# MarwanNour/SEAL-FYP-Logistic-Regression

Measured on AMD Instinct MI355X. Metric: CKKS ciphertext rotate+plain-mult ops/sec at N=16384; HBM GB/s vs roofline, higher is better.
Workload: dtype u64; 1 GPU; C3: N=16384, coeff_modulus bits [60, 40, 40, 40, 40, 60], level L=5 (k=6); per step and per GPU 4608 independent rotate_vector(step=1, direct Galois key)+multiply_plain, uniform random residues drawn on the device, inputs resident in HBM; batch_per_gpu=4608, parallelism=1 x independent ciphertext batches (no data-path collective), algorithmic_bytes_per_op=11141120

## Files before the change

### seal_fyp_logistic_regression_amd/csrc/hefx_keyswitch.hip

```cpp
#include <cstdio>
#include <cstdlib>
#include "hefx_internal.h"
#include "hefx_ntt.cuh"
#include "hefx_ntt8.cuh"

template <int LOGN>
struct KsWaves {
    static constexpr int INV = LOGN <= 14 ? 2 : 4;
    static constexpr int FWD = LOGN <= 13 ? 2 : 4;
    static constexpr int NB_INV = (INV <= 2 && LOGN <= 13) ? 1 : 2, NB_FWD = (FWD <= 2 && LOGN < 13) ? 1 : 2;
};

namespace hefx {

typedef u64 u64x2_t __attribute__((ext_vector_type(2)));
__device__ __forceinline__ ulonglong2 nt_load16(const u64 *p)
{
    const u64x2_t v = __builtin_nontemporal_load(reinterpret_cast<const u64x2_t *>(p));
    return make_ulonglong2(v.x, v.y);
}
__device__ __forceinline__ void nt_store16(u64 *p, u64 a, u64 b)
{
    u64x2_t v;
    v.x = a, v.y = b;
    __builtin_nontemporal_store(v, reinterpret_cast<u64x2_t *>(p));
}

template <int LOGN>
struct SplitCfg {
    using C = NttCfg<LOGN - 1>;
    static constexpr int N = 1 << LOGN;
    static constexpr int H = N / 2;
    static constexpr int T = C::T;
    static constexpr size_t LDS_BYTES = sizeof(u64) * C::LDS_WORDS;
};

__host__ __device__ static inline int split_grid(int rows) { return ((rows + 7) / 8) * 16; }
__device__ static __forceinline__ void split_decode(int bid, int &p, int &h)
{
    h = (bid >> 3) & 1;
    p = ((bid >> 4) << 3) | (bid & 7);
}
__host__ __device__ static inline int group_grid(int groups, int fan) { return ((groups + 7) / 8) * 2 * fan * 8; }
// ... 83 lines not shown
    extern __shared__ __align__(16) u64 lds[];
    int p, h;
    split_decode(blockIdx.x, p, h);
    if (p >= rows || (!noperm && ks_gated_out(S))) return;
    intt_digits_body<LOGN>(T, items[p / L], L, relin, noperm, p / L, p % L, h, S, lds);
}

#ifndef HEFX_SMALL_MAX
#define HEFX_SMALL_MAX 32
#endif
constexpr int KS_SMALL_MAX = HEFX_SMALL_MAX;
struct KsSmallItems {
    KsItem it[KS_SMALL_MAX];
};
static_assert(sizeof(KsSmallItems) + sizeof(DevTables) + sizeof(KsScratch) + sizeof(void *) + 8 * sizeof(int) <= 4096,
              "small-batch descriptors no longer fit the 4 KiB kernel-argument segment: lower HEFX_SMALL_MAX");
template <int LOGN>
__global__ __launch_bounds__(SplitCfg<LOGN>::T, KsWaves<LOGN>::INV) void ks_intt_digits_small_kernel(DevTables T, KsSmallItems small,
                                                                                    KsItem *__restrict__ items_out, int n,
                                                                                    int L, int relin, int rows, KsScratch S)
{
    extern __shared__ __align__(16) u64 lds[];
    HEFX_STAMP_KERNEL(0);
    HEFX_STAMP_AT(0);
    if (blockIdx.x == 0 && (int)threadIdx.x < n) items_out[threadIdx.x] = small.it[threadIdx.x];
    int p, h;
    split_decode(blockIdx.x, p, h);
    if (p >= rows) return;
    intt_digits_body<LOGN>(T, small.it[p / L], L, relin, 0, p / L, p % L, h, S, lds);
    HEFX_STAMP_AT(15);
}

__device__ __forceinline__ bool slot_is_f64(const DevTables &T, int L, int jj);
template <int LOGN>
__device__ __forceinline__ void ntt_digit_row(const DevTables &T, int L, int rows, int stream_x, const KsScratch &S,
                                              u64 *lds)
{
    using SC = SplitCfg<LOGN>;
    using C = typename SC::C;
    int g, jj, h;
    if (stream_x & 2) {
        const int x = blockIdx.x & 7, rest = blockIdx.x >> 3;
        const int nsg = (rows + 7) >> 3;
        const int sg = rest % nsg, slot = rest / nsg;
        g = sg * 8 + x;
        h = slot & 1;
        const int rank = slot >> 1, di = g % L;
        int heavy = 0;
        for (int mm = 0; mm < L; ++mm) heavy += !slot_is_f64(T, L, mm >= di ? mm + 1 : mm);
        int want = rank < heavy ? rank : rank - heavy;
        jj = 0;
        for (int mm = 0; mm < L; ++mm) {
            const bool hv = !slot_is_f64(T, L, mm >= di ? mm + 1 : mm);
            if (hv == (rank < heavy)) {
                if (want == 0) {
                    jj = mm;
                    break;
                }
                --want;
            }
        }
    } else
        group_decode(blockIdx.x, L, g, jj, h);
    if (g >= rows || (S.gate_mode == 2 && ks_gated_out(S))) return;
    const int t = threadIdx.x;
    const int b = g / L, i = g % L;
    if (jj >= i) ++jj;
    const int m = jj < L ? jj : T.k - 1;
    const ModConst mc = T.mods[m];
    const u64 qi = T.mods[i].q;
    const u64 *__restrict__ dd = S.d + ((size_t)b * L + i) * SC::N;
    u64 v[16];
    const InMode mode = {qi > mc.q, T.modsf[i].q == 0.0, false, 0};
    const int tl = HEFX_EO_LANE(SC, t);
    auto ld = [&](int r, u64 &x, u64 &y) {
        const uint32_t e = eo_nat<SC>(tl, r);
        x = dd[e];
        y = dd[e + SC::H / 2];
    };
    const ModConstF mf = T.modsf[m];
    split_fwd<LOGN, KsWaves<LOGN>::NB_FWD, true>(v, ld, mode, lds, ntt_tables(T, m), mc, mf, t, h, tl,
                                                 mac_x_slack(mc, mf, L));
    u64 *__restrict__ xd = S.x + (((size_t)b * L + i) * (L + 1) + jj) * SC::N + (size_t)h * SC::H;
    if (stream_x & 1) {
#pragma unroll
        for (int r = 0; r < 16; r += 2) nt_store16(xd + C::idx_io(t, r), v[r], v[r + 1]);
    } else {
#pragma unroll
        for (int r = 0; r < 16; r += 2)
            *reinterpret_cast<ulonglong2 *>(xd + C::idx_io(t, r)) = make_ulonglong2(v[r], v[r + 1]);
    }
}

struct MacW {
    struct Ctx {
        ModConst mc;
    };
    __device__ static __forceinline__ Ctx make(const ModConst &mc, const ModConstF &) { return Ctx{mc}; }
    typedef ulonglong2 X;
    struct K {
        ulonglong2 k0, k1;
    };
    __device__ static __forceinline__ X xin(const ulonglong2 &bits, bool, const Ctx &) { return bits; }
    __device__ static __forceinline__ K kin(const ulonglong2 &k0, const ulonglong2 &k1, const Ctx &) { return K{k0, k1}; }
    u64 a0xl = 0, a0xh = 0, a0yl = 0, a0yh = 0, a1xl = 0, a1xh = 0, a1yl = 0, a1yh = 0;
    __device__ __forceinline__ void mac(const X &x, const K &k, const Ctx &)
    {
        mac128(a0xl, a0xh, x.x, k.k0.x);
        mac128(a0yl, a0yh, x.y, k.k0.y);
        mac128(a1xl, a1xh, x.x, k.k1.x);
        mac128(a1yl, a1yh, x.y, k.k1.y);
    }
    __device__ __forceinline__ void mac_diag(const MacW &in, const ulonglong2 &dg, const Ctx &c)
    {
        ulonglong2 r0, r1;
        in.result(r0, r1, c);
        mac128(a0xl, a0xh, r0.x, dg.x);
        mac128(a0yl, a0yh, r0.y, dg.y);
        mac128(a1xl, a1xh, r1.x, dg.x);
        mac128(a1yl, a1yh, r1.y, dg.y);
    }
    template <bool LT2Q = false>
    __device__ __forceinline__ void result_data(ulonglong2 &r0, ulonglong2 &r1, const Ctx &c) const { result<LT2Q>(r0, r1, c); }
    template <bool LT2Q = false>
    __device__ __forceinline__ void result(ulonglong2 &r0, ulonglong2 &r1, const Ctx &c) const
    {
        r0.x = LT2Q ? barrett128_lt2q(a0xl, a0xh, c.mc) : barrett128(a0xl, a0xh, c.mc);
        r0.y = LT2Q ? barrett128_lt2q(a0yl, a0yh, c.mc) : barrett128(a0yl, a0yh, c.mc);
        r1.x = LT2Q ? barrett128_lt2q(a1xl, a1xh, c.mc) : barrett128(a1xl, a1xh, c.mc);
        r1.y = LT2Q ? barrett128_lt2q(a1yl, a1yh, c.mc) : barrett128(a1yl, a1yh, c.mc);
    }
};

struct MacL {
    typedef MacW::Ctx Ctx;
    __device__ static __forceinline__ Ctx make(const ModConst &mc, const ModConstF &) { return Ctx{mc}; }
    struct X {
        uint32_t xl, xh, yl, yh;
    };
    struct K {
        uint32_t k0xl, k0xh, k0yl, k0yh, k1xl, k1xh, k1yl, k1yh;
    };
    __device__ static __forceinline__ uint32_t lo30(u64 v) { return (uint32_t)v & 0x3FFFFFFFu; }
    __device__ static __forceinline__ uint32_t hi30(u64 v) { return (uint32_t)(v >> 30); }
    __device__ static __forceinline__ X xin(const ulonglong2 &b, bool, const Ctx &)
    {
        return X{lo30(b.x), hi30(b.x), lo30(b.y), hi30(b.y)};
    }
    __device__ static __forceinline__ K kin(const ulonglong2 &k0, const ulonglong2 &k1, const Ctx &)
    {
        return K{lo30(k0.x), hi30(k0.x), lo30(k0.y), hi30(k0.y), lo30(k1.x), hi30(k1.x), lo30(k1.y), hi30(k1.y)};
    }
    u64 c[4][3] = {};
    __device__ static __forceinline__ void mad(u64 (&col)[3], uint32_t xl, uint32_t xh, uint32_t kl, uint32_t kh)
    {
        col[0] += (u64)xl * kl;
        col[1] += (u64)xl * kh;
        col[1] += (u64)xh * kl;
        col[2] += (u64)xh * kh;
    }
    __device__ __forceinline__ void mac(const X &x, const K &k, const Ctx &)
    {
        mad(c[0], x.xl, x.xh, k.k0xl, k.k0xh);
        mad(c[1], x.yl, x.yh, k.k0yl, k.k0yh);
        mad(c[2], x.xl, x.xh, k.k1xl, k.k1xh);
        mad(c[3], x.yl, x.yh, k.k1yl, k.k1yh);
    }
    __device__ __forceinline__ void mac_diag(const MacL &in, const ulonglong2 &dg, const Ctx &cx)
    {
        ulonglong2 r0, r1;
        in.result(r0, r1, cx);
        const uint32_t dxl = lo30(dg.x), dxh = hi30(dg.x), dyl = lo30(dg.y), dyh = hi30(dg.y);
        mad(c[0], lo30(r0.x), hi30(r0.x), dxl, dxh);
        mad(c[1], lo30(r0.y), hi30(r0.y), dyl, dyh);
        mad(c[2], lo30(r1.x), hi30(r1.x), dxl, dxh);
        mad(c[3], lo30(r1.y), hi30(r1.y), dyl, dyh);
    }
    template <bool LT2Q>
    __device__ static __forceinline__ u64 fold(const u64 (&col)[3], const ModConst &mc)
    {
        u64 lo = col[0], hi = 0, t = col[1] << 30;
        lo += t;
        hi += (col[1] >> 34) + (lo < t);
        t = col[2] << 60;
        lo += t;
        hi += (col[2] >> 4) + (lo < t);
        return LT2Q ? barrett128_lt2q(lo, hi, mc) : barrett128(lo, hi, mc);
    }
    template <bool LT2Q = false>
    __device__ __forceinline__ void result_data(ulonglong2 &r0, ulonglong2 &r1, const Ctx &cx) const { result<LT2Q>(r0, r1, cx); }
    template <bool LT2Q = false>
    __device__ __forceinline__ void result(ulonglong2 &r0, ulonglong2 &r1, const Ctx &cx) const
    {
        r0.x = fold<LT2Q>(c[0], cx.mc);
        r0.y = fold<LT2Q>(c[1], cx.mc);
        r1.x = fold<LT2Q>(c[2], cx.mc);
        r1.y = fold<LT2Q>(c[3], cx.mc);
    }
};

struct MacF {
    typedef ArithF64::Ctx Ctx;
    __device__ static __forceinline__ Ctx make(const ModConst &, const ModConstF &mf) { return ArithF64::make(mf); }
    typedef double2 X;
    struct K {
        double k0x, k0y, k1x, k1y;
    };
    __device__ static __forceinline__ X xin(const ulonglong2 &b, bool own, const Ctx &)
    {
        return own ? make_double2(ArithF64::from_u64(b.x), ArithF64::from_u64(b.y))
                   : make_double2(__longlong_as_double((long long)b.x), __longlong_as_double((long long)b.y));
    }
    __device__ static __forceinline__ K kin(const ulonglong2 &k0, const ulonglong2 &k1, const Ctx &)
    {
        return K{ArithF64::from_u64(k0.x), ArithF64::from_u64(k0.y), ArithF64::from_u64(k1.x), ArithF64::from_u64(k1.y)};
    }
    double a0x = 0.0, a0y = 0.0, a1x = 0.0, a1y = 0.0;
    __device__ __forceinline__ void mac(const X &x, const K &k, const Ctx &c)
    {
        a0x += ArithF64::mm(x.x, k.k0x, c);
        a0y += ArithF64::mm(x.y, k.k0y, c);
        a1x += ArithF64::mm(x.x, k.k1x, c);
        a1y += ArithF64::mm(x.y, k.k1y, c);
    }
    __device__ __forceinline__ void mac_diag(const MacF &in, const ulonglong2 &dg, const Ctx &c)
    {
        const double dx = ArithF64::from_u64(dg.x), dy = ArithF64::from_u64(dg.y);
        a0x += ArithF64::mm(in.a0x, dx, c);
        a0y += ArithF64::mm(in.a0y, dy, c);
        a1x += ArithF64::mm(in.a1x, dx, c);
        a1y += ArithF64::mm(in.a1y, dy, c);
    }
    template <bool LT2Q = false>
    __device__ __forceinline__ void result_data(ulonglong2 &r0, ulonglong2 &r1, const Ctx &) const
    {
        r0.x = ArithF64::raw(a0x), r0.y = ArithF64::raw(a0y), r1.x = ArithF64::raw(a1x), r1.y = ArithF64::raw(a1y);
    }
    template <bool LT2Q = false>
    __device__ __forceinline__ void result(ulonglong2 &r0, ulonglong2 &r1, const Ctx &c) const
    {
        r0.x = ArithF64::canon(a0x, c);
        r0.y = ArithF64::canon(a0y, c);
        r1.x = ArithF64::canon(a1x, c);
        r1.y = ArithF64::canon(a1y, c);
    }
};

__device__ __forceinline__ bool slot_is_f64(const DevTables &T, int L, int jj)
{
    return T.modsf[jj < L ? jj : T.k - 1].q != 0.0;
}

template <class F>
__device__ __forceinline__ void mac_dispatch(const DevTables &T, int m, int L, const F &f)
{
    if (T.modsf[m].q != 0.0)
        f(MacF());
    else if (L <= 8 && (T.mods[m].q >> 60) == 0)
        f(MacL());
    else
        f(MacW());
}

template <bool STREAM>
__device__ __forceinline__ void mac_store(u64 *acc0, u64 *acc1, size_t w, const ulonglong2 &r0, const ulonglong2 &r1)
{
    if (STREAM) {
        nt_store16(acc0 + 2 * w, r0.x, r0.y);
        nt_store16(acc1 + 2 * w, r1.x, r1.y);
    } else {
        gst16(acc0 + 2 * w, r0);
        gst16(acc1 + 2 * w, r1);
    }
}

template <class P, int NI, bool STREAM, class XR>
__device__ __forceinline__ void mac_items(const DevTables &T, const u64 *key, int L, int jj, int m, size_t n, size_t w,
                                          const u64 *const (&own)[NI], const uint32_t (&own_elt)[NI], const XR &xrow,
                                          u64 *const (&acc0)[NI], u64 *const (&acc1)[NI])
{
    const typename P::Ctx cx = P::make(T.mods[m], T.modsf[m]);
    const int logn = T.logn;
    const size_t kpoly = (size_t)T.k * n;
    P A[NI];
    auto load_k = [&](int i, ulonglong2 &k0, ulonglong2 &k1) {
        const u64 *kb = key + ((size_t)i * 2 * T.k + m) * n;
        k0 = gld16(kb + 2 * w);
        k1 = gld16(kb + kpoly + 2 * w);
    };
    auto load_x = [&](int i, ulonglong2 (&xb)[NI]) {
#pragma unroll
        for (int e = 0; e < NI; ++e) {
            const u64 *xp = xrow(e, i) + 2 * w;
            xb[e] = STREAM ? nt_load16(xp) : gld16(xp);
        }
    };
    if (jj < L) {
        ulonglong2 xb[NI], k0, k1;
#pragma unroll
        for (int e = 0; e < NI; ++e) xb[e] = gather_pair(own[e], (uint32_t)w, own_elt[e], logn);
        load_k(jj, k0, k1);
        const typename P::K k = P::kin(k0, k1, cx);
#pragma unroll
        for (int e = 0; e < NI; ++e) A[e].mac(P::xin(xb[e], true, cx), k, cx);
    }
    constexpr int G = 1;
    auto digit_at = [&](int r) { return r < jj ? r : r + 1; };
    const int nd = jj < L ? L - 1 : L;
    int r0 = 0;
    for (; r0 + G <= nd; r0 += G) {
        ulonglong2 xb[G][NI], k0[G], k1[G];
#pragma unroll
        for (int g = 0; g < G; ++g) {
            load_x(digit_at(r0 + g), xb[g]);
            load_k(digit_at(r0 + g), k0[g], k1[g]);
        }
        HEFX_STAGE_FENCE();
#pragma unroll
        for (int g = 0; g < G; ++g) {
            const typename P::K k = P::kin(k0[g], k1[g], cx);
#pragma unroll
            for (int e = 0; e < NI; ++e) A[e].mac(P::xin(xb[g][e], false, cx), k, cx);
        }
    }
    for (; r0 < nd; ++r0) {
        ulonglong2 xb[NI], k0, k1;
        load_x(digit_at(r0), xb);
        load_k(digit_at(r0), k0, k1);
        const typename P::K k = P::kin(k0, k1, cx);
#pragma unroll
        for (int e = 0; e < NI; ++e) A[e].mac(P::xin(xb[e], false, cx), k, cx);
    }
#pragma unroll
    for (int e = 0; e < NI; ++e) {
        ulonglong2 r0, r1;
        if (jj < L)
            A[e].template result_data<true>(r0, r1, cx);
        else
            A[e].template result<true>(r0, r1, cx);
        mac_store<STREAM>(acc0[e], acc1[e], w, r0, r1);
    }
}

template <bool STREAM>
__device__ __forceinline__ void mac_unit(const DevTables &T, const KsItem *__restrict__ items, int L, int relin, int count,
                                         const KsScratch &S, int jj, int bl0, size_t w)
{
    const size_t n = (size_t)1 << T.logn;
    const int m = jj < L ? jj : T.k - 1;
    const bool two = bl0 + 1 < count;
    const KsItem it0 = items[bl0], it1 = items[bl0 + (two ? 1 : 0)];
    const int ownrow = jj < L ? jj : 0;
    const u64 *const own[2] = {it0.c_in + ((size_t)(relin ? 2 * L : L) + ownrow) * n,
                               it1.c_in + ((size_t)(relin ? 2 * L : L) + ownrow) * n};
    const uint32_t own_elt[2] = {relin ? 1u : item_elt(it0), relin ? 1u : item_elt(it1)};
    auto xrow2 = [&](int e, int i) { return S.x + (((size_t)(bl0 + e) * L + i) * (L + 1) + jj) * n; };
    auto accrow = [&](int bl, int c) { return S.acc + (((size_t)bl * 2 + c) * (L + 1) + jj) * n; };
    u64 *const acc0[2] = {accrow(bl0, 0), accrow(bl0 + 1, 0)}, *const acc1[2] = {accrow(bl0, 1), accrow(bl0 + 1, 1)};
    mac_dispatch(T, m, L, [&](auto pol) {
        using P = decltype(pol);
        if (two && it1.key == it0.key) {
            mac_items<P, 2, STREAM>(T, it0.key, L, jj, m, n, w, own, own_elt, xrow2, acc0, acc1);
        } else {
            const u64 *const o0[1] = {own[0]}, *const o1[1] = {own[1]};
            const uint32_t e0[1] = {own_elt[0]}, e1[1] = {own_elt[1]};
            u64 *const a00[1] = {acc0[0]}, *const a01[1] = {acc1[0]}, *const a10[1] = {acc0[1]}, *const a11[1] = {acc1[1]};
            mac_items<P, 1, STREAM>(T, it0.key, L, jj, m, n, w, o0, e0, [&](int, int i) { return xrow2(0, i); }, a00, a01);
            if (two)
                mac_items<P, 1, STREAM>(T, it1.key, L, jj, m, n, w, o1, e1, [&](int, int i) { return xrow2(1, i); }, a10, a11);
        }
    });
}

template <bool STREAM>
__global__ __launch_bounds__(256) void ks_mac_kernel(DevTables T, const KsItem *__restrict__ items, int L, int relin,
                                                     int count, KsScratch S)
{
    if (S.gate_mode == 2 && ks_gated_out(S)) return;
    const int jj = blockIdx.y;
#ifdef HEFX_STAMP
    const int wg = blockIdx.x + gridDim.x * (blockIdx.y + gridDim.y * blockIdx.z);
    if (threadIdx.x == 0 && wg < 1024) hefx_stamp_buf[((size_t)2 * 1024 + wg) * 16] = wall_clock64();
#endif
    mac_unit<STREAM>(T, items, L, relin, count, S, jj, 2 * blockIdx.z, (size_t)blockIdx.x * blockDim.x + threadIdx.x);
#ifdef HEFX_STAMP
    if (HEFX_STAMP > 1) asm volatile("s_waitcnt vmcnt(0) lgkmcnt(0)" ::: "memory");
    if (threadIdx.x == 0 && wg < 1024) hefx_stamp_buf[((size_t)2 * 1024 + wg) * 16 + 15] = wall_clock64();
#endif
}

template <int LOGN>
__global__ __launch_bounds__(SplitCfg<LOGN>::T, KsWaves<LOGN>::FWD) void ks_ntt_digits_kernel(DevTables T, int L, int rows,
                                                                             int stream_x, KsScratch S)
{
    extern __shared__ __align__(16) u64 lds[];
    HEFX_STAMP_KERNEL(1);
    HEFX_STAMP_AT(0);
    ntt_digit_row<LOGN>(T, L, rows, stream_x, S, lds);
    HEFX_STAMP_AT(15);
}

template <class P>
__device__ __forceinline__ void mac_gathered(P &A, const typename P::Ctx &cx, const DevTables &T, const KsItem &it,
                                             const u64 *__restrict__ c1, const KsScratch &S, int L, int jj, int m,
                                             size_t n, size_t w)
{
    const uint2 pi = gld_u32x2(it.perm + 2 * w);
    for (int i = 0; i < L; ++i) {
        const u64 *__restrict__ xrow = i == jj ? c1 + (size_t)i * n : S.x + ((size_t)i * (L + 1) + jj) * n;
        ulonglong2 xb;
        xb.x = gld8(xrow + pi.x);
        xb.y = gld8(xrow + pi.y);
        const u64 *kbase = it.key + ((size_t)i * 2 * T.k + m) * n;
        const ulonglong2 k0 = gld16(kbase + 2 * w);
        const ulonglong2 k1 = gld16(kbase + (size_t)T.k * n + 2 * w);
        A.mac(P::xin(xb, i == jj, cx), P::kin(k0, k1, cx), cx);
    }
}

__global__ __launch_bounds__(256) void ks_mac_exact_kernel(DevTables T, const KsItem *__restrict__ items, int L, KsScratch S)
{
    const size_t n = (size_t)1 << T.logn;
    const int jj = blockIdx.y, b = blockIdx.z;
    const int m = jj < L ? jj : T.k - 1;
    const size_t w = (size_t)blockIdx.x * blockDim.x + threadIdx.x;
    const KsItem it = items[b];
    if (w == 0 && jj == 0 && b == 0 && *S.gate == S.gate_tag) atomicAdd(S.gate_hits, 1u);
    const u64 *__restrict__ c1 = it.c_in + (size_t)L * n;
    const u64 *__restrict__ xs = S.x + (size_t)it.dsrc * L * (L + 1) * n;
    mac_dispatch(T, m, L, [&](auto pol) {
        using P = decltype(pol);
// ... 822 lines not shown
    }
}

template <int LOGN>
__global__ __launch_bounds__(256) void ks_pair_finish_kernel(DevTables T, const KsItem *__restrict__ items, int L, int relin,
                                                            KsScratch S)
{
    const int row = blockIdx.y, b = blockIdx.z;
    const int c = row / L, j = row % L;
    const uint32_t g = blockIdx.x * blockDim.x + threadIdx.x;
#ifdef HEFX_STAMP
    const int wg = blockIdx.x + gridDim.x * (blockIdx.y + gridDim.y * blockIdx.z);
    if (threadIdx.x == 0 && wg < 1024) hefx_stamp_buf[((size_t)5 * 1024 + wg) * 16] = wall_clock64();
#endif
    const KsItem it = items[b];
    const ModConst mc = T.mods[j];
    fwd_policy_dispatch(mc, T.modsf[j], [&](auto pol) {
        using A = decltype(pol);
        pair_finish_body<LOGN, A>(T, it, L, relin, b, c, j, g, S);
    });
#ifdef HEFX_STAMP
    if (HEFX_STAMP > 1) asm volatile("s_waitcnt vmcnt(0) lgkmcnt(0)" ::: "memory");
    if (threadIdx.x == 0 && wg < 1024) hefx_stamp_buf[((size_t)5 * 1024 + wg) * 16 + 15] = wall_clock64();
#endif
}

template <typename K>
static void set_lds(K kernel, size_t bytes)
{
    (void)hipFuncSetAttribute(reinterpret_cast<const void *>(kernel), hipFuncAttributeMaxDynamicSharedMemorySize,
                              (int)bytes);
}

template <int LOGN>
static hipError_t launch_keyswitch_chunk_t(const DevTables &T, int L, int n, const KsItem *batch, bool relin,
                                           const KsScratch &scr, bool alias, const KsSmallItems *small, int quarter,
                                           hipStream_t s, KsProf *prof, int nsrc)
{
    using SC = SplitCfg<LOGN>;
    const size_t lds = SC::LDS_BYTES;
    static PerDeviceOnce attr_once;
    if (attr_once.first()) {
        set_lds(ks_intt_digits_kernel<LOGN>, lds);
        set_lds(ks_intt_digits_small_kernel<LOGN>, lds);
        set_lds(ks_ntt_digits_kernel<LOGN>, lds);
        set_lds(ks_moddown_intt_kernel<LOGN>, lds);
        set_lds(ks_moddown_finish_kernel<LOGN>, lds);
        if (getenv("HEFX_DEBUG")) {
            int nb = -1;
            (void)hipOccupancyMaxActiveBlocksPerMultiprocessor(&nb, ks_ntt_digits_kernel<LOGN>, SC::T, lds);
            fprintf(stderr, "[hefx] ks_ntt_digits_kernel<%d>: %d threads, %zu B LDS -> %d workgroups/CU\n", LOGN, SC::T,
                    lds, nb);
        }
    }
    const int rl = relin ? 1 : 0;
    auto mark = [&](int stage) {
        if (prof && prof->used < prof->cap) {
            (void)hipEventRecord(prof->ev[prof->used], s);
            prof->stage[prof->used++] = stage;
        }
    };
    if (nsrc > 0) {
        KsScratch hs = scr, fb = scr;
        hs.gate_mode = 1;
        fb.gate_mode = 2;
        mark(1);
        hipLaunchKernelGGL((ks_intt_digits_kernel<LOGN>), dim3(split_grid(nsrc * L)), dim3(SC::T), lds, s, T, batch + n, L,
                           0, 1, nsrc * L, hs);
        mark(2);
        hipLaunchKernelGGL((ks_ntt_digits_kernel<LOGN>), dim3(group_grid(nsrc * L, L)), dim3(SC::T), lds, s, T, L, nsrc * L, 0,
                           hs);
        mark(3);
        hipLaunchKernelGGL(ks_mac_exact_kernel, dim3(SC::N / 2 / 256, L + 1, n), dim3(256), 0, s, T, batch, L, hs);
        mark(4);
        hipLaunchKernelGGL((ks_moddown_intt_kernel<LOGN>), dim3(split_grid(n * 2)), dim3(SC::T), lds, s, T, L, n * 2, hs);
        mark(5);
        hipLaunchKernelGGL((ks_moddown_finish_kernel<LOGN>), dim3(group_grid(n * 2, L)), dim3(SC::T), lds, s, T, batch, L,
                           0, n * 2, hs);
        mark(7);
        hipLaunchKernelGGL((ks_intt_digits_kernel<LOGN>), dim3(split_grid(n * L)), dim3(SC::T), lds, s, T, batch, L, 0, 0,
                           n * L, fb);
        hipLaunchKernelGGL((ks_ntt_digits_kernel<LOGN>), dim3(group_grid(n * L, L)), dim3(SC::T), lds, s, T, L, n * L, 0, fb);
        hipLaunchKernelGGL(ks_mac_kernel<false>, dim3(SC::N / 2 / 256, L + 1, (n + 1) / 2), dim3(256), 0, s, T, batch, L, 0, n,
                           fb);
        hipLaunchKernelGGL((ks_moddown_intt_kernel<LOGN>), dim3(split_grid(n * 2)), dim3(SC::T), lds, s, T, L, n * 2, fb);
// ... 13 lines not shown
        mark(1);
        hipLaunchKernelGGL((ks_pair_digits_kernel<LOGN>), fan_grid(n * L, 4 * L), dim3(TQ), ldsq, s, T, *small,
                           const_cast<KsItem *>(batch), n, L, rl, n * L, scr);
        mark(3);
        hipLaunchKernelGGL((ks_pair_mac_kernel<LOGN>), dim3(SC::N / 4 / 256, 2 * (L + 1), n), dim3(256), 0, s, T, batch, L, rl,
                           scr);
        mark(4);
        hipLaunchKernelGGL((ks_pair_moddown_kernel<LOGN>), fan_grid(n * 2, 4 * L), dim3(TQ), ldsq, s, T, L, n * 2,
                           scr);
        mark(5);
        hipLaunchKernelGGL((ks_pair_finish_kernel<LOGN>), dim3(SC::N / 4 / 256, 2 * L, n), dim3(256), 0, s, T, batch, L, rl,
                           scr);
        mark(-1);
        return hipGetLastError();
    }
    const int heavy_order = n * L * L * 2 <= 640 ? 2 : 0;
    if (small && (quarter & KS_Q_ALL)) {
        static PerDeviceOnce attrq;
        const size_t ldsq = QuarterCfg<LOGN>::LDS_BYTES;
        if (attrq.first()) {
            set_lds(ks_intt_digits_q_kernel<LOGN>, ldsq);
            set_lds(ks_ntt_digits_q_kernel<LOGN>, ldsq);
            set_lds(ks_moddown_intt_q_kernel<LOGN>, ldsq);
            set_lds(ks_moddown_finish_q_kernel<LOGN>, ldsq);
        }
        constexpr int TQ = QuarterCfg<LOGN>::T;
        mark(1);
        if (quarter & KS_Q_INTT)
            hipLaunchKernelGGL((ks_intt_digits_q_kernel<LOGN>), dim3(quarter_grid(n * L)), dim3(TQ), ldsq, s, T, *small,
                               const_cast<KsItem *>(batch), n, L, rl, n * L, scr);
        else
            hipLaunchKernelGGL((ks_intt_digits_small_kernel<LOGN>), dim3(split_grid(n * L)), dim3(SC::T), lds, s, T, *small,
                               const_cast<KsItem *>(batch), n, L, rl, n * L, scr);
        mark(2);
        if (quarter & KS_Q_NTT)
            hipLaunchKernelGGL((ks_ntt_digits_q_kernel<LOGN>), fan_grid(n * L, 4 * L), dim3(TQ), ldsq, s, T, L,
                               n * L, scr);
        else
            hipLaunchKernelGGL((ks_ntt_digits_kernel<LOGN>), dim3(group_grid(n * L, L)), dim3(SC::T), lds, s, T, L,
                               n * L, heavy_order, scr);
        mark(3);
        hipLaunchKernelGGL(ks_mac_kernel<false>, dim3(SC::N / 2 / 256, L + 1, (n + 1) / 2), dim3(256), 0, s, T, batch, L, rl, n,
                           scr);
        mark(4);
        if (quarter & KS_Q_MDI)
            hipLaunchKernelGGL((ks_moddown_intt_q_kernel<LOGN>), dim3(quarter_grid(n * 2)), dim3(TQ), ldsq, s, T, L, n * 2,
                               scr);
        else
            hipLaunchKernelGGL((ks_moddown_intt_kernel<LOGN>), dim3(split_grid(n * 2)), dim3(SC::T), lds, s, T, L, n * 2,
                               scr);
        mark(5);
        if (quarter & KS_Q_FIN)
            hipLaunchKernelGGL((ks_moddown_finish_q_kernel<LOGN>), fan_grid(n * 2, 4 * L), dim3(TQ), ldsq, s, T,
                               batch, L, rl, n * 2, scr);
        else
            hipLaunchKernelGGL((ks_moddown_finish_kernel<LOGN>), dim3(group_grid(n * 2, L)), dim3(SC::T), lds, s, T,
                               batch, L, rl, n * 2, scr);
        mark(-1);
        return hipGetLastError();
    }
    if (alias) {
        mark(0);
        hipLaunchKernelGGL(ks_alias_copy_kernel, dim3(SC::N / 2 / 256, 2 * L, n), dim3(256), 0, s, T, batch, L);
    }
    mark(1);
    if (small)
        hipLaunchKernelGGL((ks_intt_digits_small_kernel<LOGN>), dim3(split_grid(n * L)), dim3(SC::T), lds, s, T, *small,
                           const_cast<KsItem *>(batch), n, L, rl, n * L, scr);
    else
        hipLaunchKernelGGL((ks_intt_digits_kernel<LOGN>), dim3(split_grid(n * L)), dim3(SC::T), lds, s, T, batch, L, rl, 0,
                           n * L, scr);
    mark(2);
    const int stream_x = (size_t)n * L * (L + 1) * SC::N * 8 > ((size_t)256 << 20) ? 1 : 0;
    hipLaunchKernelGGL((ks_ntt_digits_kernel<LOGN>), dim3(group_grid(n * L, L)), dim3(SC::T), lds, s, T, L, n * L,
                       stream_x | heavy_order, scr);
    mark(3);
    if (stream_x)
        hipLaunchKernelGGL(ks_mac_kernel<true>, dim3(SC::N / 2 / 256, L + 1, (n + 1) / 2), dim3(256), 0, s, T, batch, L, rl, n,
                           scr);
    else
        hipLaunchKernelGGL(ks_mac_kernel<false>, dim3(SC::N / 2 / 256, L + 1, (n + 1) / 2), dim3(256), 0, s, T, batch, L, rl, n,
                           scr);
    mark(4);
    hipLaunchKernelGGL((ks_moddown_intt_kernel<LOGN>), dim3(split_grid(n * 2)), dim3(SC::T), lds, s, T, L, n * 2, scr);
    mark(5);
    hipLaunchKernelGGL((ks_moddown_finish_kernel<LOGN>), dim3(group_grid(n * 2, L)), dim3(SC::T), lds, s, T, batch, L,
                       rl, n * 2, scr);
    mark(-1);
    return hipGetLastError();
}

__global__ __launch_bounds__(256) void lt2_reduce_kernel(DevTables T, int L, int period, int rows, int chunks,
                                                         const u64 *__restrict__ partial, const u64 *addin, u64 *out)
{
    const size_t n = (size_t)1 << T.logn;
    const int r = blockIdx.y;
    const int jj = r % period;
    const u64 q = T.mods[jj < L ? jj : T.k - 1].q;
    const size_t w = (size_t)blockIdx.x * blockDim.x + threadIdx.x;
    ulonglong2 acc = addin ? reinterpret_cast<const ulonglong2 *>(addin + (size_t)r * n)[w] : make_ulonglong2(0, 0);
    for (int ch = 0; ch < chunks; ++ch) {
        const ulonglong2 v = reinterpret_cast<const ulonglong2 *>(partial + ((size_t)ch * rows + r) * n)[w];
        acc.x = addmod(acc.x, v.x, q);
        acc.y = addmod(acc.y, v.y, q);
    }
    if (period == L + 1 && jj < L && T.modsf[jj].q != 0.0)
        acc = make_ulonglong2(ArithF64::raw(ArithF64::from_u64(acc.x)), ArithF64::raw(ArithF64::from_u64(acc.y)));
    reinterpret_cast<ulonglong2 *>(out + (size_t)r * n)[w] = acc;
}

template <int LOGN>
static hipError_t launch_lt2_decompose_t(const DevTables &T, int L, const KsItem *src_item, const KsItem *rot_items,
                                         int nrot, const KsScratch &scr, const u64 *ct_new, u64 *partial_s,
                                         u64 *partial_c0, u64 *cbuf, hipStream_t s)
{
// ... 265 lines not shown
```

### seal_fyp_logistic_regression_amd/csrc/hefx_ntt.cuh

```cuda
#pragma once
#include <type_traits>

#include "hefx_modarith.cuh"

#ifdef HEFX_STAMP
namespace hefx {
static __device__ u64 hefx_stamp_buf[8 * 1024 * 16];
__device__ __forceinline__ int &hefx_stamp_kid()
{
    __shared__ int kid;
    return kid;
}
}
#define HEFX_STAMP_KERNEL(k) do { if (threadIdx.x == 0) hefx_stamp_kid() = (k); } while (0)
#define HEFX_STAMP_AT(id)                                                                                            \
    do {                                                                                                             \
        if (HEFX_STAMP > 1) asm volatile("s_waitcnt vmcnt(0) lgkmcnt(0)" ::: "memory");                              \
        const unsigned hefx_wg_ = blockIdx.x + gridDim.x * (blockIdx.y + gridDim.y * blockIdx.z);                   \
        if (threadIdx.x == 0 && hefx_wg_ < 1024)                                                                     \
            hefx_stamp_buf[((size_t)hefx_stamp_kid() * 1024 + hefx_wg_) * 16 + (id)] = wall_clock64();               \
    } while (0)
#else
#define HEFX_STAMP_KERNEL(k) do { } while (0)
#define HEFX_STAMP_AT(id) do { } while (0)
// ... 607 lines not shown
                                            u64 *lds, const typename A::TW *__restrict__ tw,
                                            const typename A::Ctx &cx, int t, int h, int t0 = -1, int mac_slack = 0)
{
    typename A::V f[16];
    split_fwd_raw<LOGN, A, LD, NB>(f, ld, mode, mc, lds, tw, cx, t, h, NoHook(), t0);
    if (MACOP && !A::IS_F64 && mac_slack == 1) {
#pragma unroll
        for (int r = 0; r < 16; ++r) v[r] = A::template mac_operand_lazy<1>(f[r], cx);
    } else if (MACOP && !A::IS_F64 && mac_slack >= 2) {
#pragma unroll
        for (int r = 0; r < 16; ++r) v[r] = A::template mac_operand_lazy<2>(f[r], cx);
    } else {
#pragma unroll
        for (int r = 0; r < 16; ++r) v[r] = MACOP ? A::mac_operand(f[r], cx) : A::fwd_finish(f[r], cx);
    }
}

template <int LOGN, int NB = 2, bool MACOP = false, class LD>
__device__ __forceinline__ void split_fwd(u64 (&v)[16], const LD &ld, const InMode &mode, u64 *lds,
                                          const NttTables &nt, const ModConst &mc, const ModConstF &mf, int t, int h,
                                          int t0 = -1, int mac_slack = 0)
{
    if (mf.q != 0.0)
        split_fwd_a<LOGN, ArithF64, LD, NB, MACOP>(v, ld, mode, mc, lds, nt.twf, ArithF64::make(mf), t, h, t0);
    else if constexpr (MACOP)
        fwd_int_dispatch(mc, [&](auto pol) {
            using A = decltype(pol);
            split_fwd_a<LOGN, A, LD, NB, MACOP>(v, ld, mode, mc, lds, nt.tw, A::make(mc), t, h, t0, mac_slack);
        });
    else
        split_fwd_a<LOGN, ArithU64, LD, NB, MACOP>(v, ld, mode, mc, lds, nt.tw, ArithU64::make(mc), t, h, t0);
}

template <int LOGN, class A, int NB = 2, class LDP>
__device__ __forceinline__ void split_inv_a(u64 (&v)[16], const LDP &ldp, u64 *lds,
                                            const typename A::TW *__restrict__ itw, const typename A::Ctx &cx, int t,
                                            int h)
{
    using C = NttCfg<LOGN - 1>;
    constexpr int BS = 16 / NB;
    typename A::V f[16];
    constexpr bool NATREC = C::R != 1;
    auto rec = [&](int r) { return NATREC ? C::idx_nat(t, r) : C::idx_out(t, r); };
#pragma unroll
    for (int g = 0; g < NB; ++g) {
        ulonglong2 pr[BS];
#pragma unroll
        for (int r = 0; r < BS; ++r) pr[r] = ldp(rec(BS * g + r));
        if (h == 0) {
#pragma unroll
            for (int r = 0; r < BS; ++r)
                f[BS * g + r] = A::gs_half_sum(A::from_u64(pr[r].x), A::from_u64(pr[r].y), cx);
        } else {
            typename A::TW w[BS];
#pragma unroll
            for (int r = 0; r < BS; ++r) w[r] = itw[C::N + rec(BS * g + r)];
#pragma unroll
            for (int r = 0; r < BS; ++r)
                f[BS * g + r] = A::gs_half_diff(A::from_u64(pr[r].x), A::from_u64(pr[r].y), w[r], cx);
        }
        HEFX_STAGE_FENCE();
    }
    if constexpr (C::R == 0) {
        typename A::V *lf = reinterpret_cast<typename A::V *>(lds);
        const int pw = t + (t >> 4), pr = 17 * t;
#pragma unroll
// ... 36 lines not shown
```

Measured before the change: 232,700 rotate+multiply_plain ops/s.

## Split digit forward NTT by parity and fuse last butterfly into MAC

The key-switch digit NTT now runs two independent half-size NTTs per digit, one per parity half (parity_fwd), with no cross-half exchange. The final radix-2 stage is deferred into the MAC kernel: each lane swaps its value with the neighbouring lane via DPP, then applies the last Cooley-Tukey butterfly with the matching twiddle before accumulating against the key. This removes the split-NTT cross-half exchange and its LDS traffic. In exchange the MAC kernel does extra butterfly arithmetic and lane shuffles for each digit element.

```diff
diff --git a/seal_fyp_logistic_regression_amd/csrc/hefx_keyswitch.hip b/seal_fyp_logistic_regression_amd/csrc/hefx_keyswitch.hip
--- a/seal_fyp_logistic_regression_amd/csrc/hefx_keyswitch.hip
+++ b/seal_fyp_logistic_regression_amd/csrc/hefx_keyswitch.hip
@@ -9,6 +9,7 @@
     static constexpr int INV = LOGN <= 14 ? 2 : 4;
     static constexpr int FWD = LOGN <= 13 ? 2 : 4;
     static constexpr int NB_INV = (INV <= 2 && LOGN <= 13) ? 1 : 2, NB_FWD = (FWD <= 2 && LOGN < 13) ? 1 : 2;
+    static constexpr bool PARITY_CUT = true;
 };
 
 namespace hefx {
@@ -158,7 +159,8 @@
 }
 
 __device__ __forceinline__ bool slot_is_f64(const DevTables &T, int L, int jj);
-template <int LOGN>
+__device__ __forceinline__ int mac_kind(const DevTables &T, int m, int L);
+template <int LOGN, bool CUT>
 __device__ __forceinline__ void ntt_digit_row(const DevTables &T, int L, int rows, int stream_x, const KsScratch &S,
                                               u64 *lds)
 {
@@ -198,15 +200,21 @@
     const u64 *__restrict__ dd = S.d + ((size_t)b * L + i) * SC::N;
     u64 v[16];
     const InMode mode = {qi > mc.q, T.modsf[i].q == 0.0, false, 0};
-    const int tl = HEFX_EO_LANE(SC, t);
-    auto ld = [&](int r, u64 &x, u64 &y) {
-        const uint32_t e = eo_nat<SC>(tl, r);
-        x = dd[e];
-        y = dd[e + SC::H / 2];
-    };
     const ModConstF mf = T.modsf[m];
-    split_fwd<LOGN, KsWaves<LOGN>::NB_FWD, true>(v, ld, mode, lds, ntt_tables(T, m), mc, mf, t, h, tl,
-                                                 mac_x_slack(mc, mf, L));
+    if constexpr (CUT) {
+        const u64 *__restrict__ dh = dd + (size_t)h * SC::H;
+        parity_fwd<LOGN>(v, [&](int r) { return dh[C::idx_nat(t, r)]; }, mode, lds, ntt_tables(T, m), mc, mf, t,
+                         mac_kind(T, m, L));
+    } else {
+        const int tl = HEFX_EO_LANE(SC, t);
+        auto ld = [&](int r, u64 &x, u64 &y) {
+            const uint32_t e = eo_nat<SC>(tl, r);
+            x = dd[e];
+            y = dd[e + SC::H / 2];
+        };
+        split_fwd<LOGN, KsWaves<LOGN>::NB_FWD, true>(v, ld, mode, lds, ntt_tables(T, m), mc, mf, t, h, tl,
+                                                     mac_x_slack(mc, mf, L));
+    }
     u64 *__restrict__ xd = S.x + (((size_t)b * L + i) * (L + 1) + jj) * SC::N + (size_t)h * SC::H;
     if (stream_x & 1) {
 #pragma unroll
@@ -229,6 +237,14 @@
     };
     __device__ static __forceinline__ X xin(const ulonglong2 &bits, bool, const Ctx &) { return bits; }
     __device__ static __forceinline__ K kin(const ulonglong2 &k0, const ulonglong2 &k1, const Ctx &) { return K{k0, k1}; }
+    typedef ulonglong2 LTW;
+    __device__ static __forceinline__ LTW ltw(const NttTables &nt, size_t i) { return gld16(nt.tw + i); }
+    __device__ static __forceinline__ X xin_cut(u64 e, u64 o, const LTW &w, const Ctx &c, int)
+    {
+        const ArithU64::Ctx ac = ArithU64::make(c.mc);
+        ArithU64::ct(e, o, w, ac, 0);
+        return make_ulonglong2(ArithU64::fwd_finish(e, ac), ArithU64::fwd_finish(o, ac));
+    }
     u64 a0xl = 0, a0xh = 0, a0yl = 0, a0yh = 0, a1xl = 0, a1xh = 0, a1yl = 0, a1yh = 0;
     __device__ __forceinline__ void mac(const X &x, const K &k, const Ctx &)
     {
@@ -277,6 +293,21 @@
     {
         return K{lo30(k0.x), hi30(k0.x), lo30(k0.y), hi30(k0.y), lo30(k1.x), hi30(k1.x), lo30(k1.y), hi30(k1.y)};
     }
+    typedef ulonglong2 LTW;
+    __device__ static __forceinline__ LTW ltw(const NttTables &nt, size_t i) { return gld16(nt.tw + i); }
+    __device__ static __forceinline__ u64 cut_reduce(u64 x, const ArithU64L::Ctx &ac, int slack)
+    {
+        x = csubn(csubn(x, ac.n8q), ac.n4q);
+        if (slack < 2) x = csubn(x, ac.n2q);
+        if (slack < 1) x = csubn(x, ac.nq);
+        return x;
+    }
+    __device__ static __forceinline__ X xin_cut(u64 e, u64 o, const LTW &w, const Ctx &c, int slack)
+    {
+        const ArithU64L::Ctx ac = ArithU64L::make(c.mc);
+        ArithU64L::ct(e, o, w, ac, 1);
+        return xin(make_ulonglong2(cut_reduce(e, ac, slack), cut_reduce(o, ac, slack)), false, c);
+    }
     u64 c[4][3] = {};
     __device__ static __forceinline__ void mad(u64 (&col)[3], uint32_t xl, uint32_t xh, uint32_t kl, uint32_t kh)
     {
@@ -341,6 +372,14 @@
     {
         return K{ArithF64::from_u64(k0.x), ArithF64::from_u64(k0.y), ArithF64::from_u64(k1.x), ArithF64::from_u64(k1.y)};
     }
+    typedef double LTW;
+    __device__ static __forceinline__ LTW ltw(const NttTables &nt, size_t i) { return nt.twf[i]; }
+    __device__ static __forceinline__ X xin_cut(u64 e, u64 o, const LTW &w, const Ctx &c, int)
+    {
+        double x = ArithF64::unraw(e), y = ArithF64::unraw(o);
+        ArithF64::ct(x, y, w, c, 0);
+        return make_double2(x, y);
+    }
     double a0x = 0.0, a0y = 0.0, a1x = 0.0, a1y = 0.0;
     __device__ __forceinline__ void mac(const X &x, const K &k, const Ctx &c)
     {
@@ -388,6 +427,23 @@
         f(MacW());
 }
 
+__device__ __forceinline__ int mac_kind(const DevTables &T, int m, int L)
+{
+    int kind = MAC_W;
+    mac_dispatch(T, m, L, [&](auto pol) {
+        using P = decltype(pol);
+        kind = std::is_same<P, MacF>::value ? MAC_F : std::is_same<P, MacL>::value ? MAC_L : MAC_W;
+    });
+    return kind;
+}
+
+__device__ __forceinline__ u64 lane_pair_swap(u64 v)
+{
+    const int lo = __builtin_amdgcn_update_dpp(0, (int)(uint32_t)v, 0xB1, 0xF, 0xF, false);
+    const int hi = __builtin_amdgcn_update_dpp(0, (int)(uint32_t)(v >> 32), 0xB1, 0xF, 0xF, false);
+    return ((u64)(uint32_t)hi << 32) | (uint32_t)lo;
+}
+
 template <bool STREAM>
 __device__ __forceinline__ void mac_store(u64 *acc0, u64 *acc1, size_t w, const ulonglong2 &r0, const ulonglong2 &r1)
 {
@@ -400,7 +456,7 @@
     }
 }
 
-template <class P, int NI, bool STREAM, class XR>
+template <class P, int NI, bool STREAM, bool CUT, class XR>
 __device__ __forceinline__ void mac_items(const DevTables &T, const u64 *key, int L, int jj, int m, size_t n, size_t w,
                                           const u64 *const (&own)[NI], const uint32_t (&own_elt)[NI], const XR &xrow,
                                           u64 *const (&acc0)[NI], u64 *const (&acc1)[NI])
@@ -414,12 +470,24 @@
         k0 = gld16(kb + 2 * w);
         k1 = gld16(kb + kpoly + 2 * w);
     };
+    const bool odd = (w & 1) != 0;
+    const size_t xoff = CUT ? (odd ? n / 2 + w - 1 : w) : 2 * w;
     auto load_x = [&](int i, ulonglong2 (&xb)[NI]) {
 #pragma unroll
         for (int e = 0; e < NI; ++e) {
-            const u64 *xp = xrow(e, i) + 2 * w;
+            const u64 *xp = xrow(e, i) + xoff;
             xb[e] = STREAM ? nt_load16(xp) : gld16(xp);
         }
+    };
+    typename P::LTW lw = {};
+    if constexpr (CUT) lw = P::ltw(ntt_tables(T, m), n / 2 + w);
+    const int slack = CUT ? mac_x_slack(T.mods[m], T.modsf[m], L) : 0;
+    auto x_of = [&](const ulonglong2 &b) {
+        if constexpr (CUT) {
+            const u64 sx = lane_pair_swap(b.x), sy = lane_pair_swap(b.y);
+            return P::xin_cut(odd ? sy : b.x, odd ? b.y : sx, lw, cx, slack);
+        } else
+            return P::xin(b, false, cx);
     };
     if (jj < L) {
         ulonglong2 xb[NI], k0, k1;
@@ -446,7 +514,7 @@
         for (int g = 0; g < G; ++g) {
             const typename P::K k = P::kin(k0[g], k1[g], cx);
 #pragma unroll
-            for (int e = 0; e < NI; ++e) A[e].mac(P::xin(xb[g][e], false, cx), k, cx);
+            for (int e = 0; e < NI; ++e) A[e].mac(x_of(xb[g][e]), k, cx);
         }
     }
     for (; r0 < nd; ++r0) {
@@ -455,7 +523,7 @@
         load_k(digit_at(r0), k0, k1);
         const typename P::K k = P::kin(k0, k1, cx);
 #pragma unroll
-        for (int e = 0; e < NI; ++e) A[e].mac(P::xin(xb[e], false, cx), k, cx);
+        for (int e = 0; e < NI; ++e) A[e].mac(x_of(xb[e]), k, cx);
     }
 #pragma unroll
     for (int e = 0; e < NI; ++e) {
@@ -468,7 +536,7 @@
     }
 }
 
-template <bool STREAM>
+template <bool STREAM, bool CUT>
 __device__ __forceinline__ void mac_unit(const DevTables &T, const KsItem *__restrict__ items, int L, int relin, int count,
                                          const KsScratch &S, int jj, int bl0, size_t w)
 {
@@ -486,20 +554,21 @@
     mac_dispatch(T, m, L, [&](auto pol) {
         using P = decltype(pol);
         if (two && it1.key == it0.key) {
-            mac_items<P, 2, STREAM>(T, it0.key, L, jj, m, n, w, own, own_elt, xrow2, acc0, acc1);
+            mac_items<P, 2, STREAM, CUT>(T, it0.key, L, jj, m, n, w, own, own_elt, xrow2, acc0, acc1);
         } else {
             const u64 *const o0[1] = {own[0]}, *const o1[1] = {own[1]};
             const uint32_t e0[1] = {own_elt[0]}, e1[1] = {own_elt[1]};
             u64 *const a00[1] = {acc0[0]}, *const a01[1] = {acc1[0]}, *const a10[1] = {acc0[1]}, *const a11[1] = {acc1[1]};
-            mac_items<P, 1, STREAM>(T, it0.key, L, jj, m, n, w, o0, e0, [&](int, int i) { return xrow2(0, i); }, a00, a01);
+            mac_items<P, 1, STREAM, CUT>(T, it0.key, L, jj, m, n, w, o0, e0, [&](int, int i) { return xrow2(0, i); }, a00, a01);
             if (two)
-                mac_items<P, 1, STREAM>(T, it1.key, L, jj, m, n, w, o1, e1, [&](int, int i) { return xrow2(1, i); }, a10, a11);
+                mac_items<P, 1, STREAM, CUT>(T, it1.key, L, jj, m, n, w, o1, e1, [&](int, int i) { return xrow2(1, i); }, a10, a11);
         }
     });
 }
 
-template <bool STREAM>
-__global__ __launch_bounds__(256) void ks_mac_kernel(DevTables T, const KsItem *__restrict__ items, int L, int relin,
+constexpr int KS_MAC_THREADS = 256;
+template <bool STREAM, bool CUT = false>
+__global__ __launch_bounds__(KS_MAC_THREADS) void ks_mac_kernel(DevTables T, const KsItem *__restrict__ items, int L, int relin,
                                                      int count, KsScratch S)
 {
     if (S.gate_mode == 2 && ks_gated_out(S)) return;
@@ -508,21 +577,22 @@
     const int wg = blockIdx.x + gridDim.x * (blockIdx.y + gridDim.y * blockIdx.z);
     if (threadIdx.x == 0 && wg < 1024) hefx_stamp_buf[((size_t)2 * 1024 + wg) * 16] = wall_clock64();
 #endif
-    mac_unit<STREAM>(T, items, L, relin, count, S, jj, 2 * blockIdx.z, (size_t)blockIdx.x * blockDim.x + threadIdx.x);
+    static_assert(KS_MAC_THREADS % 64 == 0, "the parity cut pairs lane 2v with lane 2v+1: w and the lane share their parity");
+    mac_unit<STREAM, CUT>(T, items, L, relin, count, S, jj, 2 * blockIdx.z, (size_t)blockIdx.x * KS_MAC_THREADS + threadIdx.x);
 #ifdef HEFX_STAMP
     if (HEFX_STAMP > 1) asm volatile("s_waitcnt vmcnt(0) lgkmcnt(0)" ::: "memory");
     if (threadIdx.x == 0 && wg < 1024) hefx_stamp_buf[((size_t)2 * 1024 + wg) * 16 + 15] = wall_clock64();
 #endif
 }
 
-template <int LOGN>
+template <int LOGN, bool CUT = false>
 __global__ __launch_bounds__(SplitCfg<LOGN>::T, KsWaves<LOGN>::FWD) void ks_ntt_digits_kernel(DevTables T, int L, int rows,
                                                                              int stream_x, KsScratch S)
 {
     extern __shared__ __align__(16) u64 lds[];
     HEFX_STAMP_KERNEL(1);
     HEFX_STAMP_AT(0);
-    ntt_digit_row<LOGN>(T, L, rows, stream_x, S, lds);
+    ntt_digit_row<LOGN, CUT>(T, L, rows, stream_x, S, lds);
     HEFX_STAMP_AT(15);
 }
 
@@ -1411,6 +1481,24 @@
                               (int)bytes);
 }
 
+template <int LOGN, class MARK>
+static void launch_digits_and_mac(const DevTables &T, int L, int n, const KsItem *batch, int rl, int order_flags,
+                                  bool may_stream, const KsScratch &scr, hipStream_t s, const MARK &mark)
+{
+    using SC = SplitCfg<LOGN>;
+    constexpr bool CUT = KsWaves<LOGN>::PARITY_CUT;
+    const int stream_x = may_stream && (size_t)n * L * (L + 1) * SC::N * 8 > ((size_t)256 << 20) ? 1 : 0;
+    mark(2);
+    hipLaunchKernelGGL((ks_ntt_digits_kernel<LOGN, CUT>), dim3(group_grid(n * L, L)), dim3(SC::T), SC::LDS_BYTES, s, T, L,
+                       n * L, stream_x | order_flags, scr);
+    mark(3);
+    const dim3 grid(SC::N / 2 / 256, L + 1, (n + 1) / 2);
+    if (stream_x)
+        hipLaunchKernelGGL((ks_mac_kernel<true, CUT>), grid, dim3(256), 0, s, T, batch, L, rl, n, scr);
+    else
+        hipLaunchKernelGGL((ks_mac_kernel<false, CUT>), grid, dim3(256), 0, s, T, batch, L, rl, n, scr);
+}
+
 template <int LOGN>
 static hipError_t launch_keyswitch_chunk_t(const DevTables &T, int L, int n, const KsItem *batch, bool relin,
                                            const KsScratch &scr, bool alias, const KsSmallItems *small, int quarter,
@@ -1423,13 +1511,15 @@
         set_lds(ks_intt_digits_kernel<LOGN>, lds);
         set_lds(ks_intt_digits_small_kernel<LOGN>, lds);
         set_lds(ks_ntt_digits_kernel<LOGN>, lds);
+        set_lds(ks_ntt_digits_kernel<LOGN, KsWaves<LOGN>::PARITY_CUT>, lds);
         set_lds(ks_moddown_intt_kernel<LOGN>, lds);
         set_lds(ks_moddown_finish_kernel<LOGN>, lds);
         if (getenv("HEFX_DEBUG")) {
             int nb = -1;
-            (void)hipOccupancyMaxActiveBlocksPerMultiprocessor(&nb, ks_ntt_digits_kernel<LOGN>, SC::T, lds);
-            fprintf(stderr, "[hefx] ks_ntt_digits_kernel<%d>: %d threads, %zu B LDS -> %d workgroups/CU\n", LOGN, SC::T,
-                    lds, nb);
+            (void)hipOccupancyMaxActiveBlocksPerMultiprocessor(&nb, ks_ntt_digits_kernel<LOGN, KsWaves<LOGN>::PARITY_CUT>,
+                                                               SC::T, lds);
+            fprintf(stderr, "[hefx] ks_ntt_digits_kernel<%d, %d>: %d threads, %zu B LDS -> %d workgroups/CU\n", LOGN,
+                    (int)KsWaves<LOGN>::PARITY_CUT, SC::T, lds, nb);
         }
     }
     const int rl = relin ? 1 : 0;
@@ -1509,16 +1599,15 @@
         else
             hipLaunchKernelGGL((ks_intt_digits_small_kernel<LOGN>), dim3(split_grid(n * L)), dim3(SC::T), lds, s, T, *small,
                                const_cast<KsItem *>(batch), n, L, rl, n * L, scr);
-        mark(2);
-        if (quarter & KS_Q_NTT)
+        if (quarter & KS_Q_NTT) {
+            mark(2);
             hipLaunchKernelGGL((ks_ntt_digits_q_kernel<LOGN>), fan_grid(n * L, 4 * L), dim3(TQ), ldsq, s, T, L,
                                n * L, scr);
-        else
-            hipLaunchKernelGGL((ks_ntt_digits_kernel<LOGN>), dim3(group_grid(n * L, L)), dim3(SC::T), lds, s, T, L,
-                               n * L, heavy_order, scr);
-        mark(3);
-        hipLaunchKernelGGL(ks_mac_kernel<false>, dim3(SC::N / 2 / 256, L + 1, (n + 1) / 2), dim3(256), 0, s, T, batch, L, rl, n,
-                           scr);
+            mark(3);
+            hipLaunchKernelGGL(ks_mac_kernel<false>, dim3(SC::N / 2 / 256, L + 1, (n + 1) / 2), dim3(256), 0, s, T, batch, L,
+                               rl, n, scr);
+        } else
+            launch_digits_and_mac<LOGN>(T, L, n, batch, rl, heavy_order, false, scr, s, mark);
         mark(4);
         if (quarter & KS_Q_MDI)
             hipLaunchKernelGGL((ks_moddown_intt_q_kernel<LOGN>), dim3(quarter_grid(n * 2)), dim3(TQ), ldsq, s, T, L, n * 2,
@@ -1547,17 +1636,7 @@
     else
         hipLaunchKernelGGL((ks_intt_digits_kernel<LOGN>), dim3(split_grid(n * L)), dim3(SC::T), lds, s, T, batch, L, rl, 0,
                            n * L, scr);
-    mark(2);
-    const int stream_x = (size_t)n * L * (L + 1) * SC::N * 8 > ((size_t)256 << 20) ? 1 : 0;
-    hipLaunchKernelGGL((ks_ntt_digits_kernel<LOGN>), dim3(group_grid(n * L, L)), dim3(SC::T), lds, s, T, L, n * L,
-                       stream_x | heavy_order, scr);
-    mark(3);
-    if (stream_x)
-        hipLaunchKernelGGL(ks_mac_kernel<true>, dim3(SC::N / 2 / 256, L + 1, (n + 1) / 2), dim3(256), 0, s, T, batch, L, rl, n,
-                           scr);
-    else
-        hipLaunchKernelGGL(ks_mac_kernel<false>, dim3(SC::N / 2 / 256, L + 1, (n + 1) / 2), dim3(256), 0, s, T, batch, L, rl, n,
-                           scr);
+    launch_digits_and_mac<LOGN>(T, L, n, batch, rl, heavy_order, true, scr, s, mark);
     mark(4);
     hipLaunchKernelGGL((ks_moddown_intt_kernel<LOGN>), dim3(split_grid(n * 2)), dim3(SC::T), lds, s, T, L, n * 2, scr);
     mark(5);
diff --git a/seal_fyp_logistic_regression_amd/csrc/hefx_ntt.cuh b/seal_fyp_logistic_regression_amd/csrc/hefx_ntt.cuh
--- a/seal_fyp_logistic_regression_amd/csrc/hefx_ntt.cuh
+++ b/seal_fyp_logistic_regression_amd/csrc/hefx_ntt.cuh
@@ -663,6 +663,63 @@
         split_fwd_a<LOGN, ArithU64, LD, NB, MACOP>(v, ld, mode, mc, lds, nt.tw, ArithU64::make(mc), t, h, t0);
 }
 
+template <int LOGN, class A, class LD>
+__device__ __forceinline__ void parity_fwd_raw(typename A::V (&f)[16], const LD &ld, const InMode &mode,
+                                               const ModConst &mc, u64 *lds, const typename A::TW *__restrict__ tw,
+                                               const typename A::Ctx &cx, int t)
+{
+    u64 x[16];
+#pragma unroll
+    for (int r = 0; r < 16; ++r) x[r] = ld(r);
+    if (A::IS_F64 ? mode.red_f64 : mode.red_int) {
+#pragma unroll
+        for (int r = 0; r < 16; ++r) f[r] = A::template input<1>(x[r], mode, cx, mc);
+    } else {
+#pragma unroll
+        for (int r = 0; r < 16; ++r) f[r] = A::template input<0>(x[r], mode, cx, mc);
+    }
+    ntt_fwd_core<LOGN - 1, A>(f, reinterpret_cast<typename A::V *>(lds), tw, cx, t, 1);
+    using C = NttCfg<LOGN - 1>;
+    if constexpr (C::R == 0) {
+        typename A::V *lf = reinterpret_cast<typename A::V *>(lds);
+        const int pw = 17 * t, pr = 2 * t + (t >> 3);
+#pragma unroll
+        for (int r = 0; r < 16; ++r) lf[pw + r] = f[r];
+        __syncthreads();
+#pragma unroll
+        for (int r = 0; r < 16; ++r) f[r] = lf[pr + (2 * C::T + C::T / 8) * (r >> 1) + (r & 1)];
+    }
+}
+
+enum { MAC_F = 0, MAC_L = 1, MAC_W = 2 };
+template <int LOGN, class A, class LD>
+__device__ __forceinline__ void parity_fwd_a(u64 (&v)[16], const LD &ld, const InMode &mode, const ModConst &mc, u64 *lds,
+                                             const typename A::TW *__restrict__ tw, const typename A::Ctx &cx, int t,
+                                             int kind)
+{
+    typename A::V f[16];
+    parity_fwd_raw<LOGN, A, LD>(f, ld, mode, mc, lds, tw, cx, t);
+    if (A::IS_F64 || kind == MAC_L) {
+#pragma unroll
+        for (int r = 0; r < 16; ++r) v[r] = A::raw(f[r]);
+    } else {
+#pragma unroll
+        for (int r = 0; r < 16; ++r) v[r] = A::fwd_finish(f[r], cx);
+    }
+}
+template <int LOGN, class LD>
+__device__ __forceinline__ void parity_fwd(u64 (&v)[16], const LD &ld, const InMode &mode, u64 *lds, const NttTables &nt,
+                                           const ModConst &mc, const ModConstF &mf, int t, int kind)
+{
+    if (mf.q != 0.0)
+        parity_fwd_a<LOGN, ArithF64, LD>(v, ld, mode, mc, lds, nt.twf, ArithF64::make(mf), t, kind);
+    else
+        fwd_int_dispatch(mc, [&](auto pol) {
+            using A = decltype(pol);
+            parity_fwd_a<LOGN, A, LD>(v, ld, mode, mc, lds, nt.tw, A::make(mc), t, kind);
+        });
+}
+
 template <int LOGN, class A, int NB = 2, class LDP>
 __device__ __forceinline__ void split_inv_a(u64 (&v)[16], const LDP &ldp, u64 *lds,
                                             const typename A::TW *__restrict__ itw, const typename A::Ctx &cx, int t,
```

Result: faster. 238,900 rotate+multiply_plain ops/s, median of 6 (+2.6%).
